# ltiao/bore

Hardware: AMD Instinct MI355X
Metric: BO-iterations/sec (fit+argmax), 16-16-1 MLP (higher is better)
Workload: dtype f32; 1 GPU; BASELINE config 4 (= config 1 x independent loops): Branin-2D, 16-16-1 MLP, q=0.25, 200 epochs, batch 64, 3 L-BFGS-B restarts from 1024 samples; loops_per_gpu=512, total_loops=512, schedule=async, N_start=15, N_end=217, parallelism=replica-shard x1

## Files before the change

bore_amd/csrc/bore_hip.hip:

```cpp
#include <hip/hip_runtime.h>

#include <cmath>
#include <cstdlib>
#include <cstring>

#include "host_common.h"
#include "mlp_device.h"
#include "mlp_regs.h"
#include "fit_bf16_mfma.h"
#include "arg_bf16_mfma.h"

using namespace bore;

#ifdef BORE_STAMPS
__device__ long long g_stamps[64];
#define BORE_STAMP(i)                                                                  \
  do {                                                                                 \
    if (blockIdx.x == 0 && (tid & 63) == 0 && e == 1 && s == 0) g_stamps[16 * (tid >> 6) + (i)] = clock64(); \
  } while (0)
extern "C" int bore_debug_stamps(long long *out) {
  return (int)hipMemcpyFromSymbol(out, HIP_SYMBOL(g_stamps), sizeof(long long) * 64);
}
__device__ int g_stamp_on;
#define BORE_TSTAMP(i)                                                                         \
// ... 11 lines not shown
#define FIT_MARK_DECL long long fm_last = clock64()
#define FIT_MARK(i)                                                                                    \
  do {                                                                                                 \
    const long long fm_now = clock64();                                                                \
    if ((threadIdx.x & 63) == 0) {                                                                     \
      __hip_atomic_fetch_add(&g_fit_lds[(threadIdx.x >> 6) & 7][i], (unsigned)(fm_now - fm_last), __ATOMIC_RELAXED, __HIP_MEMORY_SCOPE_WORKGROUP); \
      __hip_atomic_fetch_add(&g_fit_lds[(threadIdx.x >> 6) & 7][16 + (i)], 1u, __ATOMIC_RELAXED, __HIP_MEMORY_SCOPE_WORKGROUP); \
    }                                                                                                  \
    fm_last = fm_now;                                                                                  \
  } while (0)
extern "C" int bore_debug_fit_marks(unsigned long long *out, int reset) {
  int rc = (int)hipMemcpyFromSymbol(out, HIP_SYMBOL(g_fit_acc), sizeof(unsigned long long) * 256);
  if (reset) {
    unsigned long long z[256] = {0};
    rc |= (int)hipMemcpyToSymbol(HIP_SYMBOL(g_fit_acc), z, sizeof(z));
  }
  return rc;
}
#else
#define FIT_MARK_DECL
#define FIT_MARK(i)
#endif

#ifdef BORE_WIDE_STAMPS
__device__ long long g_wstamps[4][16];
#define BORE_WSTAMP_DECL long long ws_t = clock64(); (void)ws_t
#define BORE_WSTAMP(i)                                                   \
  do {                                                                   \
    if (blockIdx.x == 0 && (threadIdx.x & 63) == 0) {                    \
      const long long ws_n = clock64();                                  \
      g_wstamps[threadIdx.x >> 6][(i)] += ws_n - ws_t;                   \
      ws_t = ws_n;                                                       \
    }                                                                    \
  } while (0)
extern "C" int bore_debug_wide_stamps(long long *out, int reset) {
  int rc = (int)hipMemcpyFromSymbol(out, HIP_SYMBOL(g_wstamps), sizeof(long long) * 64);
  if (reset) {
    long long z[64] = {0};
    rc |= (int)hipMemcpyToSymbol(HIP_SYMBOL(g_wstamps), z, sizeof(z));
  }
  return rc;
}
#else
#define BORE_WSTAMP_DECL
#define BORE_WSTAMP(i)
#endif

extern "C" int bore_abi_version(void) { return BORE_ABI_VERSION; }
#ifndef BORE_SRC_DIGEST
#define BORE_SRC_DIGEST "unknown"
#endif
extern "C" const char *bore_source_digest(void) { return BORE_SRC_DIGEST; }

extern "C" void bore_set_batch(const bore_batch *batch) {
  if (batch) {
    g_batch_store = *batch;
    g_batch = &g_batch_store;
  } else {
    g_batch = nullptr;
  }
}
extern "C" const char *bore_last_error(void) { return g_bore_err; }

extern "C" int64_t bore_param_count(const bore_mlp_desc *desc) {
  MlpLayout L;
  if (bore_make_layout(desc, 0, 1, &L)) return fail(BORE_E_INVALID, "bad bore_mlp_desc");
  return L.P;
}

struct FitArgs {
  MlpLayout L;
  float *theta, *am, *av;
  long long *at;
  const float *X, *z;
  const int *perm;
  float *epoch_loss;
  unsigned long long seed;
  long long model0, epoch0;
  int N, epochs, B;
  float lr, beta1, beta2, eps;
  int state_in_lds, data_in_lds;
  int perm_in_lds;
  int perm_ahead;
  int o_tile, o_zt, o_misc, o_stage, o_m, o_v, o_perm, o_perm2, o_keys, o_X, o_z, o_g, o_layout, total;
  const int *ids, *its;
  int n_init;
  long long cap;
};

__device__ __forceinline__ void dw_task(const MlpLayout &L, float *smem, int o_tile, int o_m,
                                        int o_v, int l, int kb, int cb, int r_lo, int r_hi,
                                        bool want_bias, bool transposed, int kch, float alpha,
                                        float omb1, float omb2, float eps) {
  const int lane = threadIdx.x & 63, m16 = lane & 15, q4 = lane >> 4;
  float *th = smem, *tile = smem + o_tile, *sm = smem + o_m, *sv = smem + o_v;
  const int K = L.w[l - 1], Nw = L.w[l], ldw = L.ldw[l];
  const int lda_p = L.lda[l - 1], ldd = L.lda[l];
  const float *ap = tile + L.aoff[l - 1] + q4 * lda_p + kb * 16 + m16;
  const float *bp = tile + L.doff[l] + q4 * ldd + cb * 16 + m16;
  float av[4 * (BORE_BATCH_MAX / 16)], bv[4 * (BORE_BATCH_MAX / 16)];
  FIT_MARK_DECL;
  BORE_TSTAMP(8);
#pragma unroll
  for (int kc = 0; kc < kch; ++kc) {
    av[kc] = ap[kc * 4 * lda_p];
    bv[kc] = bp[kc * 4 * ldd];
  }
  int li[5];
  bool ok[5];
  const int col = cb * 16 + m16;
  if (transposed) {
    const bool is_b = want_bias && lane == 16;
    li[0] = is_b ? L.boff[l] : L.woff[l] + (kb * 16 + m16) * ldw;
    ok[0] = is_b || (q4 == 0 && kb * 16 + m16 < K);
  } else {
#pragma unroll
    for (int r = 0; r < 4; ++r) {
      li[r] = L.woff[l] + (kb * 16 + q4 * 4 + r) * ldw + col;
      ok[r] = col < Nw && kb * 16 + q4 * 4 + r < K;
    }
    li[4] = L.boff[l] + col;
    ok[4] = q4 == 0 && col < Nw;
  }
  float w[5], mm[5], vv[5];
#pragma unroll
  for (int r = 0; r < 5; ++r) {
    const bool used = transposed ? r == 0 : (r == 4 ? want_bias : (r >= r_lo && r < r_hi));
    if (!used) continue;
    w[r] = th[li[r]];
    mm[r] = sm[li[r]];
    vv[r] = sv[li[r]];
  }
  __builtin_amdgcn_sched_barrier(0);
  BORE_TSTAMP(9);
  FIT_MARK(8);
  f32x4 acc = {0.f, 0.f, 0.f, 0.f};
  float bsum = 0.f;
#pragma unroll
  for (int kc = 0; kc < kch; ++kc) {
    acc = transposed ? __builtin_amdgcn_mfma_f32_16x16x4f32(bv[kc], av[kc], acc, 0, 0, 0)
                     : __builtin_amdgcn_mfma_f32_16x16x4f32(av[kc], bv[kc], acc, 0, 0, 0);
    bsum += bv[kc];
  }
  float g[5] = {acc[0], acc[1], acc[2], acc[3], 0.f};
  BORE_TSTAMP(10);
  FIT_MARK(9);
  if (want_bias) {
    const float gb = rows_sum4(bsum);
    if (transposed) g[0] = lane == 16 ? gb : g[0];
    else g[4] = gb;
  }
  float wn[5];
#pragma unroll
  for (int r = 0; r < 5; ++r) {
    const bool used = transposed ? r == 0 : (r == 4 ? want_bias : (r >= r_lo && r < r_hi));
    if (!used) continue;
    wn[r] = adam_update(w[r], g[r], mm[r], vv[r], alpha, omb1, omb2, eps);
  }
#pragma unroll
  for (int r = 0; r < 5; ++r) {
    const bool used = transposed ? r == 0 : (r == 4 ? want_bias : (r >= r_lo && r < r_hi));
    if (!used) continue;
    if (!ok[r]) continue;
    th[li[r]] = wn[r];
    sm[li[r]] = mm[r];
    sv[li[r]] = vv[r];
  }
  BORE_TSTAMP(11);
  FIT_MARK(10);
}

template <int SHAPE, int NBLK>
__device__ __forceinline__ void dw_adam_static(const FitArgs &a, float *smem, float alpha,
                                               float omb1, float omb2) {
  constexpr MlpLayout L = bore_static_layout(SHAPE, 1, BORE_BATCH_MAX);
  constexpr int KCH = 4 * NBLK;
  int n_tiles = 0;
#pragma unroll
  for (int l = 1; l <= L.n_layers; ++l) n_tiles += (L.Np[l - 1] >> 4) * (L.Np[l] >> 4);
  const bool split = n_tiles < BORE_THREADS / 64;
  const int wv = __builtin_amdgcn_readfirstlane((int)(threadIdx.x >> 6));
  const int wmask = __builtin_amdgcn_readfirstlane((int)(blockDim.x >> 6)) - 1;
  int t = 0;
#pragma unroll
  for (int l = 1; l <= L.n_layers; ++l) {
    const int nkb = L.Np[l - 1] >> 4, ncb = L.Np[l] >> 4;
#pragma unroll
    for (int kb = 0; kb < nkb; ++kb)
#pragma unroll
      for (int cb = 0; cb < ncb; ++cb) {
        const bool transposed = L.w[l] == 1;
        const bool two = !transposed && split && L.w[l - 1] - kb * 16 > 2;
        if ((t & wmask) == wv)
          dw_task(L, smem, a.o_tile, a.o_m, a.o_v, l, kb, cb, 0,
                  two ? 2 : (L.w[l - 1] - kb * 16 < 4 ? L.w[l - 1] - kb * 16 : 4), kb == 0 && !two, transposed,
                  KCH, alpha, omb1, omb2, a.eps);
        ++t;
        if (two) {
          if ((t & wmask) == wv)
            dw_task(L, smem, a.o_tile, a.o_m, a.o_v, l, kb, cb, 2, 4, kb == 0, false, KCH, alpha,
                    omb1, omb2, a.eps);
          ++t;
        }
      }
  }
}

struct WideTile {
  int K, Nw, ldw, lda_p, ldd, aoff, doff, kb, cb;
  int li[5], gi[5];
  bool ok[5], transposed, want_bias;
};

template <int SHAPE>
__device__ __forceinline__ WideTile wide_tile(int t, int lane_in = -1) {
  constexpr MlpLayout L = bore_static_layout(SHAPE, 1, BORE_BATCH_MAX);
  const int lane = lane_in >= 0 ? lane_in : (int)(threadIdx.x & 63), m16 = lane & 15, q4 = lane >> 4;
  WideTile w;
  int woff = 0, boff = 0, goff_w = 0, goff_b = 0, ncb = 1, r = t, start = 0;
  w.K = w.Nw = w.ldw = w.lda_p = w.ldd = w.aoff = w.doff = 0;
#pragma unroll
  for (int l = 1; l <= L.n_layers; ++l) {
    const int nt = (L.Np[l - 1] >> 4) * (L.Np[l] >> 4);
    if (t >= start && t < start + nt) {
      w.K = L.w[l - 1]; w.Nw = L.w[l]; w.ldw = L.ldw[l]; w.lda_p = L.lda[l - 1]; w.ldd = L.lda[l];
      w.aoff = L.aoff[l - 1]; w.doff = L.doff[l]; woff = L.woff[l]; boff = L.boff[l];
      goff_w = L.goff_w[l]; goff_b = L.goff_b[l]; ncb = L.Np[l] >> 4; r = t - start;
    }
    start += nt;
  }
  w.kb = r / ncb;
  w.cb = r - w.kb * ncb;
  w.transposed = w.Nw == 1;
  w.want_bias = w.kb == 0;
  const int col = w.cb * 16 + m16;
  if (w.transposed) {
    const bool is_b = w.want_bias && lane == 16;
    w.li[0] = is_b ? boff : woff + (w.kb * 16 + m16) * w.ldw;
    w.gi[0] = is_b ? goff_b : goff_w + (w.kb * 16 + m16) * w.Nw;
    w.ok[0] = is_b || (q4 == 0 && w.kb * 16 + m16 < w.K);
#pragma unroll
    for (int q = 1; q < 5; ++q) { w.li[q] = w.li[0]; w.gi[q] = w.gi[0]; w.ok[q] = false; }
  } else {
#pragma unroll
    for (int q = 0; q < 4; ++q) {
      w.li[q] = woff + (w.kb * 16 + q4 * 4 + q) * w.ldw + col;
      w.gi[q] = goff_w + (w.kb * 16 + q4 * 4 + q) * w.Nw + col;
      w.ok[q] = col < w.Nw && w.kb * 16 + q4 * 4 + q < w.K;
    }
    w.li[4] = boff + col;
    w.gi[4] = goff_b + col;
    w.ok[4] = w.want_bias && q4 == 0 && col < w.Nw;
  }
  return w;
}

template <int SHAPE>
constexpr int wide_total_tiles() {
  constexpr MlpLayout L = bore_static_layout(SHAPE, 1, BORE_BATCH_MAX);
  int total = 0;
  for (int l = 1; l <= L.n_layers; ++l) total += (L.Np[l - 1] >> 4) * (L.Np[l] >> 4);
  return total;
}
template <int SHAPE>
constexpr int wide_tiles_per_wave() {
  return (wide_total_tiles<SHAPE>() + BORE_THREADS / 64 - 1) / (BORE_THREADS / 64);
}

template <int SHAPE, typename ET>
__device__ __forceinline__ void wide_grads(const ET *tile, float (&G)[wide_tiles_per_wave<SHAPE>()][5],
                                           int tid_o) {
  constexpr int KCH = BORE_BATCH_MAX / 4, TOTAL = wide_total_tiles<SHAPE>();
  constexpr int TPW = wide_tiles_per_wave<SHAPE>(), STEP = BORE_THREADS / 64;
  const int wv = __builtin_amdgcn_readfirstlane(tid_o >> 6), lane = tid_o & 63, m16 = lane & 15, q4 = lane >> 4;
  auto widen = [](ET raw) -> float {
    if constexpr (sizeof(ET) == 2) return bf16_to_f32(raw);
    else return raw;
  };
  ET av[2][KCH], bv[2][KCH];
  {
    const WideTile w0 = wide_tile<SHAPE>(wv < TOTAL ? wv : 0, lane);
    const ET *ap = tile + w0.aoff + q4 * w0.lda_p + w0.kb * 16 + m16;
    const ET *bp = tile + w0.doff + q4 * w0.ldd + w0.cb * 16 + m16;
#pragma unroll
// ... 441 lines not shown
  constexpr bool WIDE = bore_shape_is_wide(SHAPE > 0 ? SHAPE : 0);
  constexpr bool ROUNDS = bore_shape_fit_in_rounds(SHAPE > 0 ? SHAPE : 0);
  if constexpr (WIDE) {
    const long long mdl = a.ids ? uniform_i64(a.ids[slot]) : slot;
    TileOrder<WIDE ? SHAPE : 1>::convert(a.am + mdl * Lc.P, smem, true);
    TileOrder<WIDE ? SHAPE : 1>::convert(a.av + mdl * Lc.P, smem, true);
  }
  const MlpLayout &L = begin_kernel<SHAPE>(Lc, a.L, smem, a.total, a.o_layout);
  int tid = threadIdx.x;
  BORE_OPAQUE_TID(tid);
  const int nthr = blockDim.x;
  const int wv = tid >> 6, lane = tid & 63, m16 = lane & 15, q4 = lane >> 4;
  const long long model = a.ids ? uniform_i64(a.ids[slot]) : slot;
  const int P = L.P, n = layer_count<SHAPE>(L), D = L.w[0];
  const int it_cur = a.ids ? (it_now >= 0 ? it_now : uniform_i32(a.its[slot])) : 0;
  const int N = a.ids ? a.n_init + it_cur : a.N;
  const long long epoch0 = a.ids ? (long long)it_cur * a.epochs : a.epoch0;

  float *th = smem;
  float *tile = smem + a.o_tile;
  float *zt = smem + a.o_zt;
  float *misc = smem + a.o_misc;
  int *perm_all = reinterpret_cast<int *>(smem + a.o_perm);
  int *perm_s = perm_all;
  int *perm_two = reinterpret_cast<int *>(smem + a.o_perm2);
  unsigned *keys = reinterpret_cast<unsigned *>(smem + a.o_keys);
  const int PG = a.perm ? 1 : perm_group(N, BORE_THREADS);

  float *theta_g = a.theta + model * P;
  float *m_g = a.am + model * P;
  float *v_g = a.av + model * P;
  const float *X_g = a.X + model * (a.ids ? a.cap : (long long)N) * D;
  const float *z_g = a.z + model * (a.ids ? a.cap : (long long)N);
  float *sm = smem + a.o_m, *sv = smem + a.o_v;
  float *gacc = smem + a.o_g;

  load_theta(L, n, theta_g, th);
  if (a.state_in_lds) {
    load_theta(L, n, m_g, sm);
    load_theta(L, n, v_g, sv);
  }
  if (a.data_in_lds) {
    for (int i = tid; i < N * D; i += nthr) smem[a.o_X + i] = X_g[i];
    for (int i = tid; i < N; i += nthr) smem[a.o_z + i] = z_g[i];
  }
  __syncthreads();
  if (L.any_l2) {
    float reg = 0.f;
    for (int p = tid; p < P; p += nthr) {
      const ParamRef r = param_ref(L, p, n);
      const float l2 = r.k >= 0 ? L.l2_w[r.l] : L.l2_b[r.l];
      const float w = th[r.lds];
      reg = fmaf(l2 * w, w, reg);
    }
    reg = wave_sum(reg);
    if (lane == 0) atomicAdd(&misc[0], reg);
  }

  const long long t0 = a.at[model];
  AdamClock clock(a.beta1, a.beta2, t0);
  const float omb1 = 1.f - a.beta1, omb2 = 1.f - a.beta2;
  const int steps = (N + a.B - 1) / a.B;
  const bool pipe_perm = SHAPE > 0 && !WIDE && !a.perm && PG >= 2 && a.data_in_lds &&
                         ((blockDim.x == BORE_THREADS && N - (steps - 1) * a.B <= 16 * (BORE_THREADS / 64 - 1)) ||
                          (NW == 8 && blockDim.x == 2 * BORE_THREADS));
  const int draw_wave = NW == 8 && blockDim.x == 2 * BORE_THREADS ? BORE_THREADS / 64 : BORE_THREADS / 64 - 1;
  const bool ahead = NW == 8 && a.perm_ahead && !a.perm && PG == 1 && blockDim.x == 2 * BORE_THREADS;
  constexpr int PRE_KC = RegNet<(SHAPE > 0 ? SHAPE : 1), 1>::KC0;
  static_assert(WIDE || SHAPE <= 0 || (PRE_KC + 1) * BORE_THREADS <= BORE_FIT_STAGE_FLOATS_OF(SHAPE), "stage region");
  float *stage = smem + a.o_stage + (tid & (BORE_THREADS - 1));
  auto request_row = [&](float (&gx)[PRE_KC], float &gz, const int srow) {
#pragma unroll
    for (int kc = 0; kc < PRE_KC; ++kc) gx[kc] = smem[a.o_X + srow * D + min(4 * kc + q4, D - 1)];
    gz = smem[a.o_z + srow];
  };
  auto park_row = [&](const float (&gx)[PRE_KC], const float gz, const bool live_row) {
#pragma unroll
    for (int kc = 0; kc < PRE_KC; ++kc)
      stage[kc * BORE_THREADS] = (4 * kc + q4 < D && live_row) ? gx[kc] : 0.f;
    stage[PRE_KC * BORE_THREADS] = (q4 == 0 && live_row) ? gz : 0.f;
  };
  const float alpha_first = clock.advance(a.lr, a.beta1, a.beta2);
  bool first_step = true;
  __syncthreads();
#ifdef BORE_FIT_MARKS
  if (lane < 32) g_fit_lds[wv & 7][lane] = 0;
#endif
  FIT_MARK_DECL;

  if (pipe_perm) {
    make_perm_group(a.seed, a.model0 + model, epoch0, min(2, a.epochs), N, keys, perm_all);
    const bool live0 = wv * 16 + m16 < min(a.B, N);
    float gx[PRE_KC], gz;
    request_row(gx, gz, perm_all[live0 ? wv * 16 + m16 : 0]);
    if (wv < BORE_THREADS / 64) park_row(gx, gz, live0);
  }

  auto run_epochs = [&](auto pipe_c) {
  constexpr bool PIPE = decltype(pipe_c)::value;
  for (int e = 0; e < a.epochs; ++e) {
    FIT_MARK(12);
    if constexpr (PIPE) {
      perm_s = perm_all + (e & 1) * N;
    } else if (a.perm) {
      if (a.perm_in_lds) {
        const int *pg = a.perm + (model * a.epochs + e) * (long long)N;
        for (int i = tid; i < N; i += nthr) perm_s[i] = pg[i];
        __syncthreads();
      }
    } else if (PG > 1) {
      const int eg = e & (PG - 1);
      if (eg == 0)
        make_perm_group(a.seed, a.model0 + model, epoch0 + e, min(PG, a.epochs - e), N, keys,
                        perm_all);
      perm_s = perm_all + eg * N;
    } else if (ahead) {
      perm_s = (e & 1) ? perm_two : perm_all;
      if (e == 0) make_perm(shuffle_base(a.seed, a.model0 + model, epoch0), N, keys, perm_s);
    } else {
      make_perm(shuffle_base(a.seed, a.model0 + model, epoch0 + e), N, keys, perm_s);
    }
    float eloss = 0.f;
    FIT_MARK(13);

    for (int s = 0; s < steps; ++s) {
      FIT_MARK(14);
      const int row0 = s * a.B;
      const int nb = min(a.B, N - row0);
      const float inv_nb = fit_rcp((float)nb);
      const float alpha = first_step ? alpha_first : misc[5];
      first_step = false;
      float reg = 0.f;
      const int nsub = SHAPE > 0 ? 1 : (nb + BORE_BATCH_MAX - 1) / BORE_BATCH_MAX;
      for (int sub = 0; sub < nsub; ++sub) {
      const int r0 = row0 + sub * BORE_BATCH_MAX;
      const int nr = SHAPE > 0 ? nb : min(BORE_BATCH_MAX, nb - sub * BORE_BATCH_MAX);
      const bool first_sub = sub == 0, last_sub = sub + 1 == nsub;
      BORE_STAMP(0);
      FIT_MARK(7);
      FIT_MARK(11);
      BORE_WSTAMP_DECL;
      int src = 0;
      bool live_n = false;
      float cx[PRE_KC], cz = 0.f;
      if constexpr (SHAPE > 0) {
        if constexpr (PIPE) {
#pragma unroll
          for (int kc = 0; kc < PRE_KC; ++kc) cx[kc] = stage[kc * BORE_THREADS];
          cz = stage[PRE_KC * BORE_THREADS];
          const bool last_s = s == steps - 1;
          const int *perm_n = last_s ? perm_all + ((e + 1) & 1) * N : perm_s;
          const int row0n = last_s ? 0 : row0 + a.B;
          const int nbn = last_s && e + 1 >= a.epochs ? 0 : min(a.B, N - row0n);
          live_n = wv * 16 + m16 < nbn;
          src = perm_n[live_n ? row0n + wv * 16 + m16 : 0];
        } else if (wv * 16 + m16 < nb) {
          src = perm_s[row0 + wv * 16 + m16];
        }
      }
      if (wv * 16 < nr || (bore_shape_is_wide(SHAPE > 0 ? SHAPE : 0) && wv < BORE_THREADS / 64)) {
        const int rb = wv;
        if constexpr (SHAPE > 0) {
          using Net = RegNet<SHAPE, 1>;
          Net net;
          if constexpr (Net::RT_ACT) net.set_acts(a.L);
          net.load_fwd(th);
// ... 84 lines not shown
          BORE_WSTAMP(4);
        } else {
        {
          float *A0 = tile + L.aoff[0] + (rb * 16 + m16) * L.lda[0];
          const int row = rb * 16 + m16;
          const int src = row < nr ? (a.perm_in_lds ? perm_s[r0 + row]
                                                    : a.perm[(model * a.epochs + e) * (long long)N + r0 + row])
                                   : 0;
          if (a.data_in_lds) {
            for (int d = q4; d < D; d += 4) A0[d] = row < nr ? smem[a.o_X + src * D + d] : 0.f;
            if (q4 == 0) zt[row] = row < nr ? smem[a.o_z + src] : 0.f;
          } else {
            for (int d = q4; d < D; d += 4) A0[d] = row < nr ? X_g[src * D + d] : 0.f;
            if (q4 == 0) zt[row] = row < nr ? z_g[src] : 0.f;
          }
        }
        wave_lds_sync();
        fwd_all<true>(L, n, th, tile, rb, true);
        if (lane < 16) {
          const int row = rb * 16 + lane;
          float delta = 0.f;
          if (row < nr) {
            const float x = tile[L.aoff[n] + row * L.lda[n]];
            const float zz = zt[row];
            delta = fit_bce(x, zz, a.epoch_loss != nullptr, eloss) * inv_nb;
          }
          tile[L.doff[n] + row * L.lda[n]] = delta;
        }
        wave_lds_sync();
#pragma unroll
        for (int l = n; l >= 2; --l) {
          bwd_rowblock(L, th, tile, l, rb);
          wave_lds_sync();
        }
        }
        if (tid == 0 && L.any_l2 && first_sub) {
          eloss += misc[0] * (float)nb;
          misc[0] = 0.f;
        }
      } else if constexpr (PIPE) {
        if (wv < BORE_THREADS / 64) {
          float gx[PRE_KC], gz;
          request_row(gx, gz, src);
          park_row(gx, gz, live_n);
        }
        if (wv == draw_wave && s == steps - 1 && e + 2 < a.epochs) {
          long long draw_epoch = epoch0 + e + 2;
          asm volatile("" : "+v"(draw_epoch));
          if (N <= 64)
            make_perm_wave(shuffle_base(a.seed, a.model0 + model, draw_epoch), N,
                           reinterpret_cast<unsigned long long *>(keys), perm_all + (e & 1) * N);
          else
            make_perm_wave_buckets(shuffle_base(a.seed, a.model0 + model, draw_epoch), N,
                                   reinterpret_cast<unsigned long long *>(keys), perm_all + (e & 1) * N);
        }
      } else {
        if (ahead && wv == BORE_THREADS / 64 && s < 3 && first_sub && e + 1 < a.epochs) {
          long long draw_epoch = epoch0 + e + 1;
          asm volatile("" : "+v"(draw_epoch));
          make_perm_buckets<true>(shuffle_base(a.seed, a.model0 + model, draw_epoch), N, keys,
                                  ((e + 1) & 1) ? perm_two : perm_all, s, s);
        }
      }
      __syncthreads();
#ifdef BORE_STAMPS
      if (tid == 0) g_stamp_on = (e == 1 && s == 0);
      __syncthreads();
#endif
      BORE_STAMP(5);
      FIT_MARK(4);

      const int kch = (nr + 3) >> 2;
      const int wmask_g = (int)(blockDim.x >> 6) - 1;
      int t = 0;
      if constexpr (ROUNDS) {
      } else if constexpr (bore_shape_is_wide(SHAPE > 0 ? SHAPE : 0)) {
        int tid_o = tid;
        asm volatile("" : "+v"(tid_o));
        BORE_WSTAMP(5);
        wide_fused_f32<SHAPE>(th, tile, m_g, v_g, alpha, omb1, omb2, a.eps, tid_o);
        BORE_WSTAMP(6);
      } else if constexpr (SHAPE > 0) {
        switch ((nb + 15) >> 4) {
          case 1: dw_adam_static<SHAPE, 1>(a, smem, alpha, omb1, omb2); break;
          case 2: dw_adam_static<SHAPE, 2>(a, smem, alpha, omb1, omb2); break;
          case 3: dw_adam_static<SHAPE, 3>(a, smem, alpha, omb1, omb2); break;
          default: dw_adam_static<SHAPE, 4>(a, smem, alpha, omb1, omb2); break;
        }
        FIT_MARK(15);
      } else
#pragma unroll
      for (int l = 1; l <= n; ++l) {
        const int K = L.w[l - 1], Nw = L.w[l], ldw = L.ldw[l];
        const int lda_p = L.lda[l - 1], ldd = L.lda[l];
        const int nkb = L.Np[l - 1] >> 4, ncb = L.Np[l] >> 4;
#pragma unroll
        for (int kb = 0; kb < nkb; ++kb)
#pragma unroll
          for (int cb = 0; cb < ncb; ++cb, ++t) {
            if ((t & wmask_g) != wv) continue;
            const float *ap = tile + L.aoff[l - 1] + q4 * lda_p + kb * 16 + m16;
            const float *bp = tile + L.doff[l] + q4 * ldd + cb * 16 + m16;
            f32x4 acc = {0.f, 0.f, 0.f, 0.f};
            float bsum = 0.f;
            const bool want_bias = kb == 0;
            const int col = cb * 16 + m16;
            const bool cvalid = col < Nw;
            if (!first_sub) {
#pragma unroll
              for (int r = 0; r < 4; ++r) {
                const int row = kb * 16 + q4 * 4 + r;
                if (cvalid && row < K) acc[r] = gacc[L.woff[l] + row * ldw + col];
              }
            }
            float pm[4] = {0.f, 0.f, 0.f, 0.f}, pv[4] = {0.f, 0.f, 0.f, 0.f}, pmb = 0.f, pvb = 0.f;
            if (!a.state_in_lds && last_sub) {
#pragma unroll
              for (int r = 0; r < 4; ++r) {
                const int row = kb * 16 + q4 * 4 + r;
                if (cvalid && row < K) {
                  pm[r] = m_g[L.goff_w[l] + row * Nw + col];
                  pv[r] = v_g[L.goff_w[l] + row * Nw + col];
                }
              }
              if (want_bias && q4 == 0 && cvalid) {
                pmb = m_g[L.goff_b[l] + col];
                pvb = v_g[L.goff_b[l] + col];
              }
            }
            int kc = 0;
            for (; kc + 4 <= kch; kc += 4) {
              const float a0 = ap[kc * 4 * lda_p], a1 = ap[(kc + 1) * 4 * lda_p],
                          a2 = ap[(kc + 2) * 4 * lda_p], a3 = ap[(kc + 3) * 4 * lda_p];
              const float b0 = bp[kc * 4 * ldd], b1 = bp[(kc + 1) * 4 * ldd],
                          b2 = bp[(kc + 2) * 4 * ldd], b3 = bp[(kc + 3) * 4 * ldd];
              acc = __builtin_amdgcn_mfma_f32_16x16x4f32(a0, b0, acc, 0, 0, 0);
              acc = __builtin_amdgcn_mfma_f32_16x16x4f32(a1, b1, acc, 0, 0, 0);
              acc = __builtin_amdgcn_mfma_f32_16x16x4f32(a2, b2, acc, 0, 0, 0);
              acc = __builtin_amdgcn_mfma_f32_16x16x4f32(a3, b3, acc, 0, 0, 0);
              bsum = (((bsum + b0) + b1) + b2) + b3;
            }
            for (; kc < kch; ++kc) {
              const float av = ap[kc * 4 * lda_p], bv = bp[kc * 4 * ldd];
              acc = __builtin_amdgcn_mfma_f32_16x16x4f32(av, bv, acc, 0, 0, 0);
              bsum += bv;
            }
            if (!last_sub) {
#pragma unroll
              for (int r = 0; r < 4; ++r) {
                const int row = kb * 16 + q4 * 4 + r;
                if (cvalid && row < K) gacc[L.woff[l] + row * ldw + col] = acc[r];
              }
              if (want_bias) {
                const float gb = rows_sum4(bsum);
                if (q4 == 0 && cvalid)
                  gacc[L.boff[l] + col] = first_sub ? gb : gacc[L.boff[l] + col] + gb;
              }
              continue;
            }
#pragma unroll
            for (int r = 0; r < 4; ++r) {
              const int row = kb * 16 + q4 * 4 + r;
              if (cvalid && row < K) {
                const int li = L.woff[l] + row * ldw + col;
                float w = th[li];
                float g = acc[r];
                const float l2 = L.l2_w[l];
                if (l2 != 0.f) g = fmaf(2.f * l2, w, g);
                if (a.state_in_lds) {
                  float mm = sm[li], vv = sv[li];
                  w = adam_update(w, g, mm, vv, alpha, omb1, omb2, a.eps);
                  sm[li] = mm;
                  sv[li] = vv;
                } else {
                  const int gi = L.goff_w[l] + row * Nw + col;
                  float mm = pm[r], vv = pv[r];
                  w = adam_update(w, g, mm, vv, alpha, omb1, omb2, a.eps);
                  m_g[gi] = mm;
                  v_g[gi] = vv;
                }
                th[li] = w;
                if (l2 != 0.f) reg = fmaf(l2 * w, w, reg);
              }
            }
            if (want_bias) {
              const float gb = rows_sum4(bsum);
              if (q4 == 0 && cvalid) {
                const int li = L.boff[l] + col;
                float w = th[li];
                float g = first_sub ? gb : gacc[li] + gb;
                const float l2 = L.l2_b[l];
                if (l2 != 0.f) g = fmaf(2.f * l2, w, g);
                if (a.state_in_lds) {
                  float mm = sm[li], vv = sv[li];
                  w = adam_update(w, g, mm, vv, alpha, omb1, omb2, a.eps);
                  sm[li] = mm;
                  sv[li] = vv;
                } else {
                  const int gi = L.goff_b[l] + col;
                  float mm = pmb, vv = pvb;
                  w = adam_update(w, g, mm, vv, alpha, omb1, omb2, a.eps);
                  m_g[gi] = mm;
                  v_g[gi] = vv;
                }
                th[li] = w;
                if (l2 != 0.f) reg = fmaf(l2 * w, w, reg);
              }
            }
          }
      }
      if (!last_sub) __syncthreads();
      }
      if (L.any_l2) {
        reg = wave_sum(reg);
        if (lane == 0) atomicAdd(&misc[0], reg);
      }
      if (wv == (BORE_THREADS / 64) - 1) {
        const float an = clock.advance(a.lr, a.beta1, a.beta2);
        if (lane == 0) misc[5] = an;
      }
      BORE_STAMP(6);
      FIT_MARK(5);
      __syncthreads();
      BORE_STAMP(7);
      FIT_MARK(6);
    }
    if (a.epoch_loss) {
      eloss = wave_sum(eloss);
      if (lane == 0 && wv < 4) misc[1 + wv] = eloss;
      __syncthreads();
      if (tid == 0)
        a.epoch_loss[model * a.epochs + e] = (misc[1] + misc[2] + misc[3] + misc[4]) / (float)N;
    }
  }
  };
  if constexpr (SHAPE > 0 && !WIDE) {
    if (pipe_perm) run_epochs(std::true_type{});
    else run_epochs(std::false_type{});
  } else {
    run_epochs(std::false_type{});
  }

  __syncthreads();
  store_theta(L, n, th, theta_g);
  if (a.state_in_lds) {
    store_theta(L, n, sm, m_g);
    store_theta(L, n, sv, v_g);
  }
  if constexpr (WIDE) {
    __syncthreads();
    TileOrder<WIDE ? SHAPE : 1>::convert(m_g, smem, false);
    TileOrder<WIDE ? SHAPE : 1>::convert(v_g, smem, false);
  }
  if (tid == 0) a.at[model] = t0 + (long long)a.epochs * steps;
#ifdef BORE_FIT_MARKS
  if (lane < 32) atomicAdd(&g_fit_acc[wv & 7][lane], (unsigned long long)g_fit_lds[wv & 7][lane]);
#endif
}

template <int SHAPE>
__global__ __launch_bounds__(BORE_THREADS) void fit_kernel(const FitArgs a) {
  fit_body<SHAPE>(a, blockIdx.x);
}
template <int SHAPE>
__global__ __launch_bounds__(2 * BORE_THREADS) void fit_kernel_w8(const FitArgs a) {
  fit_body<SHAPE, 8>(a, blockIdx.x);
}

struct FitBf16Args {
  MlpLayout L;
  float *theta, *am, *av;
  long long *at;
  const float *X, *z;
  const int *perm;
  float *epoch_loss;
  unsigned long long seed;
  long long model0, epoch0;
  int N, epochs, B;
  float lr, beta1, beta2, eps;
  int o_tile, o_misc, o_perm, o_keys, total;
};

template <int SHAPE>
__global__ __launch_bounds__(BORE_THREADS) void fit_bf16_kernel(const FitBf16Args a) {
  extern __shared__ float smem[];
  constexpr MlpLayout L = bore_static_layout(SHAPE, 1, BORE_BATCH_MAX);
  using Net = RegNet<SHAPE, 1, true>;
  const int tid = threadIdx.x, nthr = blockDim.x;
  const int wv = tid >> 6, lane = tid & 63, m16 = lane & 15, q4 = lane >> 4;
  const long long model = blockIdx.x;
  constexpr int P = L.P, n = L.n_layers, D = L.w[0];
  const int N = a.N;
  for (int i = tid; i < (a.total >> 2); i += nthr) smem[i] = 0.f;
  __syncthreads();
  char *base = reinterpret_cast<char *>(smem);
  unsigned short *th16 = reinterpret_cast<unsigned short *>(base);
  unsigned short *tile16 = reinterpret_cast<unsigned short *>(base + a.o_tile);
  float *misc = reinterpret_cast<float *>(base + a.o_misc);
  int *perm_all = reinterpret_cast<int *>(base + a.o_perm);
  int *perm_s = perm_all;
  unsigned *keys = reinterpret_cast<unsigned *>(base + a.o_keys);
  const int PG = a.perm ? 1 : perm_group(N, BORE_THREADS);

  float *theta_g = a.theta + model * P;
  float *m_g = a.am + model * P;
  float *v_g = a.av + model * P;
  const float *X_g = a.X + model * (long long)N * D;
  const float *z_g = a.z + model * (long long)N;
  for (int p = tid; p < P; p += nthr) th16[param_ref(L, p, n).lds] = f32_to_bf16(theta_g[p]);

  const long long t0 = a.at[model];
  AdamClock clock(a.beta1, a.beta2, t0);
  const float omb1 = 1.f - a.beta1, omb2 = 1.f - a.beta2;
  const int steps = (N + a.B - 1) / a.B;
  const float alpha_first = clock.advance(a.lr, a.beta1, a.beta2);
  bool first_step = true;
  __syncthreads();
#ifdef BORE_FIT_MARKS
  if (lane < 32) g_fit_lds[wv & 7][lane] = 0;
#endif
// ... 667 lines not shown
  return rc == BORE_E_UNSUPPORTED && desc && desc->compute == BORE_COMPUTE_F32 && !g_batch;
}

static int fit_build(const bore_mlp_desc *desc, int n_models, float *theta, float *adam_m,
                     float *adam_v, int64_t *adam_t, const float *X, const float *z, int64_t N,
                     int epochs, int batch_size, const int32_t *perm, uint64_t seed,
                     int64_t model_index0, int64_t epoch0, const bore_adam_cfg *adam,
                     float *epoch_loss, FitArgs &a, size_t &lds_floats, int &shape_out) {
  if (batch_size < 1) return fail(BORE_E_INVALID, "fit: batch_size must be positive (got %d)", batch_size);
  if (N < 1 || N > (1 << 24)) return fail(BORE_E_INVALID, "fit: N=%lld out of range", (long long)N);
  const int tile_rows = batch_size < BORE_BATCH_MAX ? batch_size : BORE_BATCH_MAX;
  auto fit_flavour = [&](const bore_mlp_desc *d) {
    return g_batch ? bore_kernel_flavour(d, batch_size == BORE_BATCH_MAX) : bore_fit_flavour(d, batch_size == BORE_BATCH_MAX);
  };
  const int flavour_early = desc ? fit_flavour(desc) : 0;
  const size_t stage_f = flavour_early > 0 && !bore_shape_is_wide(flavour_early) ? BORE_FIT_STAGE_FLOATS_OF(flavour_early) : 0;
  const size_t fixed_extra = BORE_BATCH_MAX + 8 + stage_f + BORE_LAYOUT_FLOATS + 12;
  const bool rounds = desc && desc->compute != BORE_COMPUTE_BF16 && batch_size == BORE_BATCH_MAX && !g_batch &&
                      bore_shape_fit_in_rounds(bore_kernel_flavour(desc, true));
  int rc;
  if (rounds) {
    if (n_models < 1) return fail(BORE_E_INVALID, "n_models must be >= 1 (got %d)", n_models);
    if (bore_make_layout(desc, 1, BORE_BATCH_MAX, &a.L)) return fail(BORE_E_INVALID, "bad bore_mlp_desc");
    a.L.tile_floats = WideTp16<4>::total();
    const size_t need = (size_t)a.L.P_lds + a.L.tile_floats + fixed_extra + (size_t)N * (perm ? 1 : 3);
    rc = need * 4 <= BORE_LDS_BYTES ? 0 : BORE_E_UNSUPPORTED;
    if (rc) {
      const size_t avail = BORE_LDS_BYTES / 4 - ((size_t)a.L.P_lds + a.L.tile_floats + fixed_extra);
      return fail(BORE_E_UNSUPPORTED,
                  "fit: N=%lld rows exceed what one workgroup's LDS holds beside this network (the "
                  "epoch's shuffle lives there): at most %zu rows",
                  (long long)N, avail / (perm ? 1 : 3));
    }
  } else
  rc = check_common(desc, n_models, 1, tile_rows, false, fixed_extra + (size_t)N * (perm ? 1 : 3),
                    &a.L);
  a.perm_in_lds = 1;
  if (rc == BORE_E_UNSUPPORTED && !check_common(desc, n_models, 1, tile_rows, false, fixed_extra, &a.L)) {
    if (perm && !g_batch) {
      a.perm_in_lds = 0;
      rc = 0;
    } else {
      const size_t avail = BORE_LDS_BYTES / 4 - ((size_t)a.L.P_lds + a.L.tile_floats + fixed_extra);
      return fail(g_batch ? BORE_E_UNSUPPORTED : BORE_E_NEEDS_PERM,
                  "fit: N=%lld rows exceed what one workgroup's LDS holds beside this network when the "
                  "epoch's shuffle is drawn on the device (at most %zu rows): pass explicit shuffles "
                  "(`perm`, e.g. from bore_amd.shuffle.permutations) -- any N then",
                  (long long)N, avail / 3);
    }
  }
  if (rc) return rc;
  const MlpLayout &L = a.L;
  if (L.w[L.n_layers] != 1)
    return fail(BORE_E_INVALID, "fit: the last Dense layer must have 1 unit (binary classifier)");
  if (L.act[L.n_layers] != BORE_ACT_SIGMOID && L.act[L.n_layers] != BORE_ACT_LINEAR)
    return fail(BORE_E_INVALID, "fit: BCE needs a sigmoid or linear (from_logits) output layer");
  if (!theta || !adam_m || !adam_v || !adam_t || !X || !z || !adam)
    return fail(BORE_E_INVALID, "fit: null pointer");
  if (epochs < 0) return fail(BORE_E_INVALID, "fit: epochs < 0");
  if (epochs == 0) return 1;

  a.theta = theta; a.am = adam_m; a.av = adam_v; a.at = (long long *)adam_t;
  a.X = X; a.z = z; a.perm = perm; a.epoch_loss = epoch_loss;
  a.seed = seed; a.model0 = model_index0; a.epoch0 = epoch0;
  a.N = (int)N; a.epochs = epochs; a.B = batch_size;
  a.lr = adam->lr; a.beta1 = adam->beta1; a.beta2 = adam->beta2; a.eps = adam->eps;
  a.ids = a.its = nullptr; a.n_init = 0; a.cap = 0;
  if (g_batch) {
    if (perm || epoch_loss) return fail(BORE_E_INVALID, "fit: no perm / epoch_loss in batch mode");
    a.ids = g_batch->ids; a.its = g_batch->its; a.n_init = g_batch->n_init; a.cap = g_batch->cap;
  }

  size_t off = 0;
  off += L.P_lds;
  a.o_tile = (int)off; off += L.tile_floats;
  a.o_zt = (int)off; off += BORE_BATCH_MAX;
  a.o_misc = (int)off; off += 8;
  a.o_stage = (int)off; off += stage_f;
  const int PG = perm ? 1 : perm_group(N, BORE_THREADS);
  size_t perm_f = a.perm_in_lds ? (size_t)PG * N : 0, keys_f = perm ? 0 : (size_t)perm_group_scratch_floats(N, PG);
  if (!perm && stage_f && N <= 128 && perm_f < 4 * (size_t)N) perm_f = 4 * (size_t)N;
  if (!perm && stage_f && keys_f < BORE_PERM_WAVE_FLOATS) keys_f = BORE_PERM_WAVE_FLOATS;
  a.perm_ahead = 0;
  a.o_perm2 = 0;
  if (g_batch)
    for (long long nn : {(long long)(N < 64 ? N : 64), (long long)(N < 128 ? N : 128)}) {
      const int pg = perm_group(nn, BORE_THREADS);
      if ((size_t)pg * nn > perm_f) perm_f = (size_t)pg * nn;
      if ((size_t)perm_group_scratch_floats(nn, pg) > keys_f)
        keys_f = (size_t)perm_group_scratch_floats(nn, pg);
    }
  if (g_batch && stage_f) {
    const size_t nn = N < 128 ? (size_t)N : 128;
    if (perm_f < 4 * nn) perm_f = 4 * nn;
  }
  a.o_perm = (int)off; off += perm_f;
  off = (off + 3) & ~(size_t)3;
  a.o_keys = (int)off; off += keys_f;
  a.o_g = (int)off;
  if (batch_size > BORE_BATCH_MAX) off += L.P_lds;
  if ((off + BORE_LAYOUT_FLOATS + 4) * 4 > BORE_LDS_BYTES)
    return fail(BORE_E_UNSUPPORTED, "fit: theta+tile+perm need %zu B of LDS (> %d)", off * 4,
                BORE_LDS_BYTES);
  const size_t tail = BORE_LAYOUT_FLOATS + 4;
  a.state_in_lds = (off + tail + 2 * (size_t)L.P_lds) * 4 <= BORE_LDS_BYTES;
  a.o_m = a.o_v = 0;
  if (a.state_in_lds) {
    a.o_m = (int)off; off += L.P_lds;
    a.o_v = (int)off; off += L.P_lds;
  }
  const size_t data = (size_t)N * (L.w[0] + 1);
  a.data_in_lds = (off + tail + data) * 4 <= BORE_LDS_BYTES;
  a.o_X = a.o_z = 0;
  if (a.data_in_lds) {
    a.o_X = (int)off; off += (size_t)N * L.w[0];
    a.o_z = (int)off; off += N;
  }
  {
    const int fl = fit_flavour(desc);
    if (!perm && !g_batch && a.perm_in_lds && PG == 1 && N <= 512 && batch_size <= BORE_BATCH_MAX &&
        (fl == 2 || fl == 5 || fl == BORE_FIT_SHAPE_16_32 || (fl < 0 && fl >= -4)) &&
        (off + (size_t)N + tail) * 4 <= BORE_LDS_BYTES) {
      a.perm_ahead = 1;
      a.o_perm2 = (int)off; off += (size_t)N;
    }
  }
  a.total = (int)off;
  off = (off + 3) & ~(size_t)3;
  a.o_layout = (int)off;
  const size_t off_layout = off;
  int shape = fit_flavour(desc);
  if (!a.perm_in_lds && shape > 0) {
    if (bore_shape_is_wide(shape))
      return fail(BORE_E_UNSUPPORTED, "fit: N=%lld rows with this wide network: the shuffle must fit in LDS", (long long)N);
    shape = -desc->n_layers;
  }
  if (shape > 0 && !rounds && (!bore_shape_has_static_fit(shape) || (!a.state_in_lds && !bore_shape_is_wide(shape))))
    shape = -desc->n_layers;
  if (shape > 0 && bore_shape_is_wide(shape)) {
    static_assert(WideTp<3>::total() <= bore_static_layout(3, 1, BORE_BATCH_MAX).tile_floats,
                  "the transposed images must fit the tile region");
    if (a.state_in_lds) return fail(BORE_E_UNSUPPORTED, "fit: internal: wide shape with Adam slots in LDS");
  }
  lds_floats = off_layout + (shape == 0 ? BORE_LAYOUT_FLOATS : 0);
  shape_out = shape;
  return 0;
}

static int bore_pads_to_shape(const bore_mlp_desc *d) {
  if (d->compute != BORE_COMPUTE_F32 || bore_match_shape(d)) return 0;
  for (int s : {1, 2, 5, BORE_FIT_SHAPE_16_32, BORE_FIT_SHAPE_16_16})
    if (bore_flavour_on(s) && d->input_dim < kShapes[s].D && bore_desc_matches(d, s, true, true, true)) return s;
  return 0;
}

static int fit_padded(const bore_mlp_desc *desc, int S, int n_models, float *theta, float *adam_m, float *adam_v,
                      int64_t *adam_t, const float *X, const float *z, int64_t N, int epochs, int batch_size,
                      const int32_t *perm, uint64_t seed, int64_t model_index0, int64_t epoch0,
                      const bore_adam_cfg *adam, float *epoch_loss, void *stream) {
  bore_mlp_desc dp = *desc;
  dp.input_dim = kShapes[S].D;
  const size_t D = desc->input_dim, DS = dp.input_dim, H = desc->units[0];
  const int64_t P = bore_param_count(desc), PS = bore_param_count(&dp);
  {
    FitArgs probe;
    size_t off = 0;
// ... 256 lines not shown
```

Before: 291,300 BO-iterations/s.

## Add specialized single-batch fit loop keeping Adam state in registers

Adds a dedicated epoch loop for the case where the whole dataset fits in one minibatch (N <= batch size, four waves, no L2, no loss logging). The loop runs forward and backward per row, then does the weight-gradient Adam step. When each wave owns at most one gradient tile, it keeps that tile's weights and Adam moments in registers across all epochs and flushes the moments to LDS only at the end. This is meant to cut per-epoch LDS traffic and the generic loop's overhead for small N early in each BO run. The cost is more code paths and register pressure, and the path is on by default through an environment variable that can turn it off.

```diff
diff --git a/bore_amd/csrc/bore_hip.hip b/bore_amd/csrc/bore_hip.hip
--- a/bore_amd/csrc/bore_hip.hip
+++ b/bore_amd/csrc/bore_hip.hip
@@ -117,17 +117,24 @@
   int state_in_lds, data_in_lds;
   int perm_in_lds;
   int perm_ahead;
+  int single_batch;
   int o_tile, o_zt, o_misc, o_stage, o_m, o_v, o_perm, o_perm2, o_keys, o_X, o_z, o_g, o_layout, total;
   const int *ids, *its;
   int n_init;
   long long cap;
 };
 
+struct DwSlots {
+  float w[5], m[5], v[5];
+};
+enum { DW_STEP = 0, DW_LOAD, DW_STEP_REGS, DW_FLUSH };
+template <int MODE = DW_STEP>
 __device__ __forceinline__ void dw_task(const MlpLayout &L, float *smem, int o_tile, int o_m,
                                         int o_v, int l, int kb, int cb, int r_lo, int r_hi,
                                         bool want_bias, bool transposed, int kch, float alpha,
-                                        float omb1, float omb2, float eps) {
-  const int lane = threadIdx.x & 63, m16 = lane & 15, q4 = lane >> 4;
+                                        float omb1, float omb2, float eps, DwSlots *st = nullptr,
+                                        int tx = threadIdx.x) {
+  const int lane = tx & 63, m16 = lane & 15, q4 = lane >> 4;
   float *th = smem, *tile = smem + o_tile, *sm = smem + o_m, *sv = smem + o_v;
   const int K = L.w[l - 1], Nw = L.w[l], ldw = L.ldw[l];
   const int lda_p = L.lda[l - 1], ldd = L.lda[l];
@@ -136,10 +143,12 @@
   float av[4 * (BORE_BATCH_MAX / 16)], bv[4 * (BORE_BATCH_MAX / 16)];
   FIT_MARK_DECL;
   BORE_TSTAMP(8);
-#pragma unroll
-  for (int kc = 0; kc < kch; ++kc) {
-    av[kc] = ap[kc * 4 * lda_p];
-    bv[kc] = bp[kc * 4 * ldd];
+  if constexpr (MODE == DW_STEP || MODE == DW_STEP_REGS) {
+#pragma unroll
+    for (int kc = 0; kc < kch; ++kc) {
+      av[kc] = ap[kc * 4 * lda_p];
+      bv[kc] = bp[kc * 4 * ldd];
+    }
   }
   int li[5];
   bool ok[5];
@@ -158,14 +167,34 @@
     ok[4] = q4 == 0 && col < Nw;
   }
   float w[5], mm[5], vv[5];
+  int c = 0;
 #pragma unroll
   for (int r = 0; r < 5; ++r) {
     const bool used = transposed ? r == 0 : (r == 4 ? want_bias : (r >= r_lo && r < r_hi));
     if (!used) continue;
-    w[r] = th[li[r]];
-    mm[r] = sm[li[r]];
-    vv[r] = sv[li[r]];
-  }
+    if constexpr (MODE == DW_STEP || MODE == DW_LOAD) {
+      w[r] = th[li[r]];
+      mm[r] = sm[li[r]];
+      vv[r] = sv[li[r]];
+    } else {
+      w[r] = st->w[c];
+      mm[r] = st->m[c];
+      vv[r] = st->v[c];
+    }
+    if constexpr (MODE == DW_LOAD) {
+      st->w[c] = w[r];
+      st->m[c] = mm[r];
+      st->v[c] = vv[r];
+    }
+    ++c;
+    if constexpr (MODE == DW_FLUSH) {
+      if (ok[r]) {
+        sm[li[r]] = mm[r];
+        sv[li[r]] = vv[r];
+      }
+    }
+  }
+  if constexpr (MODE == DW_LOAD || MODE == DW_FLUSH) return;
   __builtin_amdgcn_sched_barrier(0);
   BORE_TSTAMP(9);
   FIT_MARK(8);
@@ -192,10 +221,19 @@
     if (!used) continue;
     wn[r] = adam_update(w[r], g[r], mm[r], vv[r], alpha, omb1, omb2, eps);
   }
+  c = 0;
 #pragma unroll
   for (int r = 0; r < 5; ++r) {
     const bool used = transposed ? r == 0 : (r == 4 ? want_bias : (r >= r_lo && r < r_hi));
     if (!used) continue;
+    if constexpr (MODE == DW_STEP_REGS) {
+      st->w[c] = wn[r];
+      st->m[c] = mm[r];
+      st->v[c] = vv[r];
+      ++c;
+      if (ok[r]) th[li[r]] = wn[r];
+      continue;
+    }
     if (!ok[r]) continue;
     th[li[r]] = wn[r];
     sm[li[r]] = mm[r];
@@ -205,16 +243,27 @@
   FIT_MARK(10);
 }
 
-template <int SHAPE, int NBLK>
+static constexpr bool dw_one_task_per_wave(int shape) {
+  const MlpLayout L = bore_static_layout(shape, 1, BORE_BATCH_MAX);
+  int n_tiles = 0, n_tasks = 0;
+  for (int l = 1; l <= L.n_layers; ++l) n_tiles += (L.Np[l - 1] >> 4) * (L.Np[l] >> 4);
+  for (int l = 1; l <= L.n_layers; ++l)
+    for (int kb = 0; kb < (L.Np[l - 1] >> 4); ++kb)
+      n_tasks += (L.Np[l] >> 4) * (L.w[l] != 1 && n_tiles < BORE_THREADS / 64 && L.w[l - 1] - kb * 16 > 2 ? 2 : 1);
+  return n_tasks <= BORE_THREADS / 64;
+}
+
+template <int SHAPE, int NBLK, int MODE = DW_STEP>
 __device__ __forceinline__ void dw_adam_static(const FitArgs &a, float *smem, float alpha,
-                                               float omb1, float omb2) {
+                                               float omb1, float omb2, DwSlots *st = nullptr,
+                                               int tx = threadIdx.x) {
   constexpr MlpLayout L = bore_static_layout(SHAPE, 1, BORE_BATCH_MAX);
   constexpr int KCH = 4 * NBLK;
   int n_tiles = 0;
 #pragma unroll
   for (int l = 1; l <= L.n_layers; ++l) n_tiles += (L.Np[l - 1] >> 4) * (L.Np[l] >> 4);
   const bool split = n_tiles < BORE_THREADS / 64;
-  const int wv = __builtin_amdgcn_readfirstlane((int)(threadIdx.x >> 6));
+  const int wv = __builtin_amdgcn_readfirstlane(tx >> 6);
   const int wmask = __builtin_amdgcn_readfirstlane((int)(blockDim.x >> 6)) - 1;
   int t = 0;
 #pragma unroll
@@ -227,14 +276,14 @@
         const bool transposed = L.w[l] == 1;
         const bool two = !transposed && split && L.w[l - 1] - kb * 16 > 2;
         if ((t & wmask) == wv)
-          dw_task(L, smem, a.o_tile, a.o_m, a.o_v, l, kb, cb, 0,
-                  two ? 2 : (L.w[l - 1] - kb * 16 < 4 ? L.w[l - 1] - kb * 16 : 4), kb == 0 && !two, transposed,
-                  KCH, alpha, omb1, omb2, a.eps);
+          dw_task<MODE>(L, smem, a.o_tile, a.o_m, a.o_v, l, kb, cb, 0,
+                        two ? 2 : (L.w[l - 1] - kb * 16 < 4 ? L.w[l - 1] - kb * 16 : 4), kb == 0 && !two, transposed,
+                        KCH, alpha, omb1, omb2, a.eps, st, tx);
         ++t;
         if (two) {
           if ((t & wmask) == wv)
-            dw_task(L, smem, a.o_tile, a.o_m, a.o_v, l, kb, cb, 2, 4, kb == 0, false, KCH, alpha,
-                    omb1, omb2, a.eps);
+            dw_task<MODE>(L, smem, a.o_tile, a.o_m, a.o_v, l, kb, cb, 2, 4, kb == 0, false, KCH, alpha,
+                          omb1, omb2, a.eps, st, tx);
           ++t;
         }
       }
@@ -842,6 +891,12 @@
   };
   const float alpha_first = clock.advance(a.lr, a.beta1, a.beta2);
   bool first_step = true;
+  int single_nblk = 0;
+  if constexpr (SHAPE > 0 && !WIDE && NW == 4)
+    if (pipe_perm && a.single_batch && N <= a.B && a.epoch_loss == nullptr && !L.any_l2) {
+      single_nblk = __builtin_amdgcn_readfirstlane((N + 15) >> 4);
+      if (tid == 0) misc[5] = alpha_first;
+    }
   __syncthreads();
 #ifdef BORE_FIT_MARKS
   if (lane < 32) g_fit_lds[wv & 7][lane] = 0;
@@ -1092,10 +1147,10 @@
         BORE_WSTAMP(6);
       } else if constexpr (SHAPE > 0) {
         switch ((nb + 15) >> 4) {
-          case 1: dw_adam_static<SHAPE, 1>(a, smem, alpha, omb1, omb2); break;
-          case 2: dw_adam_static<SHAPE, 2>(a, smem, alpha, omb1, omb2); break;
-          case 3: dw_adam_static<SHAPE, 3>(a, smem, alpha, omb1, omb2); break;
-          default: dw_adam_static<SHAPE, 4>(a, smem, alpha, omb1, omb2); break;
+          case 1: dw_adam_static<SHAPE, 1>(a, smem, alpha, omb1, omb2, nullptr, tid); break;
+          case 2: dw_adam_static<SHAPE, 2>(a, smem, alpha, omb1, omb2, nullptr, tid); break;
+          case 3: dw_adam_static<SHAPE, 3>(a, smem, alpha, omb1, omb2, nullptr, tid); break;
+          default: dw_adam_static<SHAPE, 4>(a, smem, alpha, omb1, omb2, nullptr, tid); break;
         }
         FIT_MARK(15);
       } else
@@ -1244,8 +1299,82 @@
     }
   }
   };
+  auto run_single = [&](auto nblk_c) {
+    constexpr int NBLK = decltype(nblk_c)::value;
+    if constexpr (SHAPE > 0 && !WIDE && NW == 4) {
+      using Net = RegNet<SHAPE, 1>;
+      static_assert(Net::KC0 == PRE_KC, "the parked row has the first layer's k-chunks");
+      const int wv_s = __builtin_amdgcn_readfirstlane(wv);
+      const int row = wv * 16 + m16;
+      const bool live = row < N;
+      const float inv_nb = __int_as_float(__builtin_amdgcn_readfirstlane(__float_as_int(fit_rcp((float)N))));
+      float *A0 = tile + L.aoff[0] + row * L.lda[0];
+      constexpr bool SLOTS = dw_one_task_per_wave(SHAPE);
+      DwSlots slots = {};
+      if constexpr (SLOTS) dw_adam_static<SHAPE, NBLK, DW_LOAD>(a, smem, 0.f, omb1, omb2, &slots, tid);
+      for (int e = 0; e < a.epochs; ++e) {
+        FIT_MARK(12);
+        FIT_MARK(13);
+        FIT_MARK(14);
+        FIT_MARK(7);
+        FIT_MARK(11);
+        if (wv_s < NBLK) {
+          Net net;
+          if constexpr (Net::RT_ACT) net.set_acts(a.L);
+          net.load_fwd(th);
+          net.template load_bwd<Net::n, 2>(th);
+          float xin[PRE_KC], nx[PRE_KC], nz;
+#pragma unroll
+          for (int kc = 0; kc < PRE_KC; ++kc) xin[kc] = stage[kc * BORE_THREADS];
+          const float zz = stage[PRE_KC * BORE_THREADS];
+          const bool live_n = live && e + 1 < a.epochs;
+          request_row(nx, nz, perm_all[((e + 1) & 1) * N + (live_n ? row : 0)]);
+#pragma unroll
+          for (int kc = 0; kc < PRE_KC; ++kc)
+            if (4 * kc + q4 < D) A0[4 * kc + q4] = xin[kc];
+          __builtin_amdgcn_sched_barrier(0);
+          FIT_MARK(0);
+          net.forward(th, xin, true);
+          FIT_MARK(1);
+          net.template store_A<1, Net::n - 1>(tile, wv);
+          float delta = 0.f, no_loss = 0.f;
+          if (lane < 16 && live) delta = fit_bce(net.h[Net::n][0][0], zz, false, no_loss) * inv_nb;
+          if (lane < 16) tile[L.doff[Net::n] + row * L.lda[Net::n]] = delta;
+          net.set_output_delta(delta);
+          FIT_MARK(2);
+          net.template backward<Net::n, 2>(th);
+          net.template store_D<1, Net::n - 1>(tile, wv);
+          park_row(nx, nz, live_n);
+          FIT_MARK(3);
+        } else if (wv_s == BORE_THREADS / 64 - 1) {
+          if (e + 2 < a.epochs) {
+            long long draw_epoch = epoch0 + e + 2;
+            asm volatile("" : "+v"(draw_epoch));
+            make_perm_wave(shuffle_base(a.seed, a.model0 + model, draw_epoch), N,
+                           reinterpret_cast<unsigned long long *>(keys), perm_all + (e & 1) * N);
+          }
+        }
+        __syncthreads();
+        FIT_MARK(4);
+        const float alpha = misc[5 + (e & 1)];
+        dw_adam_static<SHAPE, NBLK, SLOTS ? DW_STEP_REGS : DW_STEP>(a, smem, alpha, omb1, omb2, &slots, tid);
+        FIT_MARK(15);
+        if (wv_s == BORE_THREADS / 64 - 1) {
+          const float an = clock.advance(a.lr, a.beta1, a.beta2);
+          if (lane == 0) misc[5 + ((e + 1) & 1)] = an;
+        }
+        FIT_MARK(5);
+        __syncthreads();
+        FIT_MARK(6);
+      }
+      if constexpr (SLOTS) dw_adam_static<SHAPE, NBLK, DW_FLUSH>(a, smem, 0.f, omb1, omb2, &slots, tid);
+    }
+  };
   if constexpr (SHAPE > 0 && !WIDE) {
-    if (pipe_perm) run_epochs(std::true_type{});
+    if (single_nblk == 1) run_single(std::integral_constant<int, 1>{});
+    else if (single_nblk == 2) run_single(std::integral_constant<int, 2>{});
+    else if (single_nblk == 3) run_single(std::integral_constant<int, 3>{});
+    else if (pipe_perm) run_epochs(std::true_type{});
     else run_epochs(std::false_type{});
   } else {
     run_epochs(std::false_type{});
@@ -2079,6 +2208,7 @@
   if (!perm && stage_f && N <= 128 && perm_f < 4 * (size_t)N) perm_f = 4 * (size_t)N;
   if (!perm && stage_f && keys_f < BORE_PERM_WAVE_FLOATS) keys_f = BORE_PERM_WAVE_FLOATS;
   a.perm_ahead = 0;
+  a.single_batch = !(getenv("BORE_FIT_SINGLE_BATCH") && !atoi(getenv("BORE_FIT_SINGLE_BATCH")));
   a.o_perm2 = 0;
   if (g_batch)
     for (long long nn : {(long long)(N < 64 ? N : 64), (long long)(N < 128 ? N : 128)}) {
```

After: 293,000 BO-iterations/s (median of 6 runs). Within noise of the previous version (+0.6%).
